# NikolaZubic/2dimageto3dmodel

Measured on NVIDIA H100. Metric: render+loss+GAN images/sec (cfg3: cfg2 render+loss at batch 32 + conv-GAN 256x256 G/D iteration, 1 G : 2 D, Adam), higher is better.
Workload: dtype tf32 (convs) / f32

## Files before the change

2dimageto3dmodel_b200/csrc/b3d_core.cu:

```cuda
#include <atomic>
#include <stdarg.h>
#include <string.h>

#include "b3d_common.cuh"

namespace b3d {
static thread_local char g_err[512] = "";
static thread_local char g_variant[256] = "";
static std::atomic<uint64_t> g_launches{0};

void set_error(const char* fmt, ...) {
    va_list ap;
    va_start(ap, fmt);
    vsnprintf(g_err, sizeof(g_err), fmt, ap);
    va_end(ap);
}
void clear_variant() { g_variant[0] = 0; }
void add_variant(const char* fmt, ...) {
    size_t n = strlen(g_variant);
    if (n + 2 >= sizeof(g_variant)) return;
    if (n) g_variant[n++] = ';';
    va_list ap;
    va_start(ap, fmt);
    vsnprintf(g_variant + n, sizeof(g_variant) - n, fmt, ap);
    va_end(ap);
}
void count_launch(int n) { g_launches.fetch_add((uint64_t)n, std::memory_order_relaxed); }
}

extern "C" {
const char* b3d_last_error(void) { return b3d::g_err; }
const char* b3d_last_variant(void) { return b3d::g_variant; }
int b3d_version(void) { return 410; }
uint64_t b3d_launch_count(void) { return b3d::g_launches.load(std::memory_order_relaxed); }
}
```

2dimageto3dmodel_b200/csrc/tc_common.cuh:

```cuda
#pragma once
#include <cuda.h>
#include <cuda_runtime.h>
#include <stdint.h>

#include "b3d_common.cuh"

namespace tc {

__device__ __forceinline__ uint32_t smem_u32(const void* p) { return (uint32_t)__cvta_generic_to_shared(p); }

__device__ __forceinline__ void mbar_init(uint64_t* bar, uint32_t count) {
    asm volatile("mbarrier.init.shared::cta.b64 [%0], %1;" ::"r"(smem_u32(bar)), "r"(count));
}
__device__ __forceinline__ void fence_barrier_init() { asm volatile("fence.mbarrier_init.release.cluster;" ::: "memory"); }
__device__ __forceinline__ void fence_proxy_async() { asm volatile("fence.proxy.async.shared::cta;" ::: "memory"); }

__device__ __forceinline__ void mbar_arrive_expect_tx(uint64_t* bar, uint32_t bytes) {
    asm volatile("mbarrier.arrive.expect_tx.shared::cta.b64 _, [%0], %1;" ::"r"(smem_u32(bar)), "r"(bytes) : "memory");
}
__device__ __forceinline__ void mbar_arrive(uint64_t* bar) {
    asm volatile("mbarrier.arrive.shared::cta.b64 _, [%0];" ::"r"(smem_u32(bar)) : "memory");
}
__device__ __forceinline__ void mbar_arrive(uint64_t* bar, uint32_t count) {
    asm volatile("mbarrier.arrive.shared::cta.b64 _, [%0], %1;" ::"r"(smem_u32(bar)), "r"(count) : "memory");
}
__device__ __forceinline__ void mbar_wait(uint64_t* bar, uint32_t parity) {
    asm volatile(
        "{\n"
        ".reg .pred p;\n"
        "WAIT_LOOP:\n"
        "mbarrier.try_wait.parity.shared::cta.b64 p, [%0], %1;\n"
        "@p bra WAIT_DONE;\n"
        "bra WAIT_LOOP;\n"
        "WAIT_DONE:\n"
        "}\n" ::"r"(smem_u32(bar)),
        "r"(parity)
        : "memory");
}
__device__ __forceinline__ void named_sync(uint32_t id, uint32_t count) {
    asm volatile("bar.sync %0, %1;" ::"r"(id), "r"(count) : "memory");
}

__device__ __forceinline__ void tma_prefetch_desc(const CUtensorMap* m) {
    asm volatile("prefetch.tensormap [%0];" ::"l"(reinterpret_cast<uint64_t>(m)) : "memory");
}
__device__ __forceinline__ void tma_load_3d(void* smem, const CUtensorMap* m, uint64_t* bar, int c0, int c1, int c2) {
    asm volatile(
        "cp.async.bulk.tensor.3d.shared::cluster.global.mbarrier::complete_tx::bytes [%0], [%1, {%3, %4, %5}], [%2];" ::"r"(
            smem_u32(smem)),
        "l"(reinterpret_cast<uint64_t>(m)), "r"(smem_u32(bar)), "r"(c0), "r"(c1), "r"(c2)
        : "memory");
}
__device__ __forceinline__ void tma_load_4d(void* smem, const CUtensorMap* m, uint64_t* bar, int c0, int c1, int c2,
                                            int c3) {
    asm volatile(
        "cp.async.bulk.tensor.4d.shared::cluster.global.mbarrier::complete_tx::bytes [%0], [%1, {%3, %4, %5, %6}], "
        "[%2];" ::"r"(smem_u32(smem)),
        "l"(reinterpret_cast<uint64_t>(m)), "r"(smem_u32(bar)), "r"(c0), "r"(c1), "r"(c2), "r"(c3)
        : "memory");
}
__device__ __forceinline__ void tma_load_5d(void* smem, const CUtensorMap* m, uint64_t* bar, int c0, int c1, int c2,
                                            int c3, int c4) {
    asm volatile(
        "cp.async.bulk.tensor.5d.shared::cluster.global.mbarrier::complete_tx::bytes [%0], [%1, {%3, %4, %5, %6, %7}], "
        "[%2];" ::"r"(smem_u32(smem)),
        "l"(reinterpret_cast<uint64_t>(m)), "r"(smem_u32(bar)), "r"(c0), "r"(c1), "r"(c2), "r"(c3), "r"(c4)
        : "memory");
}

__device__ __forceinline__ void wgmma_fence() { asm volatile("wgmma.fence.sync.aligned;" ::: "memory"); }
__device__ __forceinline__ void wgmma_commit() { asm volatile("wgmma.commit_group.sync.aligned;" ::: "memory"); }
template <int N>
__device__ __forceinline__ void wgmma_wait() { asm volatile("wgmma.wait_group.sync.aligned %0;" ::"n"(N) : "memory"); }
__device__ __forceinline__ uint32_t lds_u32(uint32_t smem_addr) {
    uint32_t v;
    asm volatile("ld.shared.b32 %0, [%1];" : "=r"(v) : "r"(smem_addr) : "memory");
    return v;
}
__device__ __forceinline__ float lds_f32(uint32_t smem_addr) {
    float v;
    asm volatile("ld.shared.f32 %0, [%1];" : "=f"(v) : "r"(smem_addr) : "memory");
    return v;
}
__device__ __forceinline__ float2 lds_f32x2(uint32_t smem_addr) {
    float2 v;
    asm volatile("ld.shared.v2.f32 {%0, %1}, [%2];" : "=f"(v.x), "=f"(v.y) : "r"(smem_addr) : "memory");
    return v;
}
template <int N>
__device__ __forceinline__ void setmaxnreg_dec() { asm volatile("setmaxnreg.dec.sync.aligned.u32 %0;" ::"n"(N)); }
template <int N>
__device__ __forceinline__ void setmaxnreg_inc() { asm volatile("setmaxnreg.inc.sync.aligned.u32 %0;" ::"n"(N)); }

template <int N>
struct Wgmma;
template <>
struct Wgmma<64> {
    __device__ __forceinline__ static void mma_rs(float (&d)[32], const uint32_t (&a)[4], uint64_t db, uint32_t accumulate) {
        asm volatile(
            "{\n"
            ".reg .pred p;\n"
            "setp.ne.b32 p, %37, 0;\n"
            "wgmma.mma_async.sync.aligned.m64n64k8.f32.tf32.tf32 "
            "{%0, %1, %2, %3, %4, %5, %6, %7, %8, %9, %10, %11, %12, %13, %14, %15, %16, %17, %18, %19, %20, %21, %22, %23, %24, %25, %26, %27, %28, %29, %30, %31}, "
            "{%32, %33, %34, %35}, %36, p, 1, 1;\n"
            "}\n"
            : "+f"(d[0]), "+f"(d[1]), "+f"(d[2]), "+f"(d[3]), "+f"(d[4]), "+f"(d[5]), "+f"(d[6]), "+f"(d[7]), "+f"(d[8]), "+f"(d[9]), "+f"(d[10]), "+f"(d[11]), "+f"(d[12]), "+f"(d[13]), "+f"(d[14]), "+f"(d[15]), "+f"(d[16]), "+f"(d[17]), "+f"(d[18]), "+f"(d[19]), "+f"(d[20]), "+f"(d[21]), "+f"(d[22]), "+f"(d[23]), "+f"(d[24]), "+f"(d[25]), "+f"(d[26]), "+f"(d[27]), "+f"(d[28]), "+f"(d[29]), "+f"(d[30]), "+f"(d[31])
            : "r"(a[0]), "r"(a[1]), "r"(a[2]), "r"(a[3]), "l"(db), "r"(accumulate));
    }
    __device__ __forceinline__ static void mma(float (&d)[32], uint64_t da, uint64_t db, uint32_t accumulate) {
        asm volatile(
            "{\n"
            ".reg .pred p;\n"
            "setp.ne.b32 p, %34, 0;\n"
            "wgmma.mma_async.sync.aligned.m64n64k8.f32.tf32.tf32 "
            "{%0, %1, %2, %3, %4, %5, %6, %7, %8, %9, %10, %11, %12, %13, %14, %15, %16, %17, %18, %19, %20, %21, %22, %23, %24, %25, %26, %27, %28, %29, %30, %31}, "
            "%32, %33, p, 1, 1;\n"
            "}\n"
            : "+f"(d[0]), "+f"(d[1]), "+f"(d[2]), "+f"(d[3]), "+f"(d[4]), "+f"(d[5]), "+f"(d[6]), "+f"(d[7]), "+f"(d[8]), "+f"(d[9]), "+f"(d[10]), "+f"(d[11]), "+f"(d[12]), "+f"(d[13]), "+f"(d[14]), "+f"(d[15]), "+f"(d[16]), "+f"(d[17]), "+f"(d[18]), "+f"(d[19]), "+f"(d[20]), "+f"(d[21]), "+f"(d[22]), "+f"(d[23]), "+f"(d[24]), "+f"(d[25]), "+f"(d[26]), "+f"(d[27]), "+f"(d[28]), "+f"(d[29]), "+f"(d[30]), "+f"(d[31])
            : "l"(da), "l"(db), "r"(accumulate));
    }
};
template <>
struct Wgmma<128> {
    __device__ __forceinline__ static void mma_rs(float (&d)[64], const uint32_t (&a)[4], uint64_t db, uint32_t accumulate) {
        asm volatile(
            "{\n"
            ".reg .pred p;\n"
            "setp.ne.b32 p, %69, 0;\n"
            "wgmma.mma_async.sync.aligned.m64n128k8.f32.tf32.tf32 "
            "{%0, %1, %2, %3, %4, %5, %6, %7, %8, %9, %10, %11, %12, %13, %14, %15, %16, %17, %18, %19, %20, %21, %22, %23, %24, %25, %26, %27, %28, %29, %30, %31, %32, %33, %34, %35, %36, %37, %38, %39, %40, %41, %42, %43, %44, %45, %46, %47, %48, %49, %50, %51, %52, %53, %54, %55, %56, %57, %58, %59, %60, %61, %62, %63}, "
            "{%64, %65, %66, %67}, %68, p, 1, 1;\n"
            "}\n"
            : "+f"(d[0]), "+f"(d[1]), "+f"(d[2]), "+f"(d[3]), "+f"(d[4]), "+f"(d[5]), "+f"(d[6]), "+f"(d[7]), "+f"(d[8]), "+f"(d[9]), "+f"(d[10]), "+f"(d[11]), "+f"(d[12]), "+f"(d[13]), "+f"(d[14]), "+f"(d[15]), "+f"(d[16]), "+f"(d[17]), "+f"(d[18]), "+f"(d[19]), "+f"(d[20]), "+f"(d[21]), "+f"(d[22]), "+f"(d[23]), "+f"(d[24]), "+f"(d[25]), "+f"(d[26]), "+f"(d[27]), "+f"(d[28]), "+f"(d[29]), "+f"(d[30]), "+f"(d[31]), "+f"(d[32]), "+f"(d[33]), "+f"(d[34]), "+f"(d[35]), "+f"(d[36]), "+f"(d[37]), "+f"(d[38]), "+f"(d[39]), "+f"(d[40]), "+f"(d[41]), "+f"(d[42]), "+f"(d[43]), "+f"(d[44]), "+f"(d[45]), "+f"(d[46]), "+f"(d[47]), "+f"(d[48]), "+f"(d[49]), "+f"(d[50]), "+f"(d[51]), "+f"(d[52]), "+f"(d[53]), "+f"(d[54]), "+f"(d[55]), "+f"(d[56]), "+f"(d[57]), "+f"(d[58]), "+f"(d[59]), "+f"(d[60]), "+f"(d[61]), "+f"(d[62]), "+f"(d[63])
            : "r"(a[0]), "r"(a[1]), "r"(a[2]), "r"(a[3]), "l"(db), "r"(accumulate));
    }
    __device__ __forceinline__ static void mma(float (&d)[64], uint64_t da, uint64_t db, uint32_t accumulate) {
        asm volatile(
            "{\n"
            ".reg .pred p;\n"
            "setp.ne.b32 p, %66, 0;\n"
            "wgmma.mma_async.sync.aligned.m64n128k8.f32.tf32.tf32 "
            "{%0, %1, %2, %3, %4, %5, %6, %7, %8, %9, %10, %11, %12, %13, %14, %15, %16, %17, %18, %19, %20, %21, %22, %23, %24, %25, %26, %27, %28, %29, %30, %31, %32, %33, %34, %35, %36, %37, %38, %39, %40, %41, %42, %43, %44, %45, %46, %47, %48, %49, %50, %51, %52, %53, %54, %55, %56, %57, %58, %59, %60, %61, %62, %63}, "
            "%64, %65, p, 1, 1;\n"
            "}\n"
            : "+f"(d[0]), "+f"(d[1]), "+f"(d[2]), "+f"(d[3]), "+f"(d[4]), "+f"(d[5]), "+f"(d[6]), "+f"(d[7]), "+f"(d[8]), "+f"(d[9]), "+f"(d[10]), "+f"(d[11]), "+f"(d[12]), "+f"(d[13]), "+f"(d[14]), "+f"(d[15]), "+f"(d[16]), "+f"(d[17]), "+f"(d[18]), "+f"(d[19]), "+f"(d[20]), "+f"(d[21]), "+f"(d[22]), "+f"(d[23]), "+f"(d[24]), "+f"(d[25]), "+f"(d[26]), "+f"(d[27]), "+f"(d[28]), "+f"(d[29]), "+f"(d[30]), "+f"(d[31]), "+f"(d[32]), "+f"(d[33]), "+f"(d[34]), "+f"(d[35]), "+f"(d[36]), "+f"(d[37]), "+f"(d[38]), "+f"(d[39]), "+f"(d[40]), "+f"(d[41]), "+f"(d[42]), "+f"(d[43]), "+f"(d[44]), "+f"(d[45]), "+f"(d[46]), "+f"(d[47]), "+f"(d[48]), "+f"(d[49]), "+f"(d[50]), "+f"(d[51]), "+f"(d[52]), "+f"(d[53]), "+f"(d[54]), "+f"(d[55]), "+f"(d[56]), "+f"(d[57]), "+f"(d[58]), "+f"(d[59]), "+f"(d[60]), "+f"(d[61]), "+f"(d[62]), "+f"(d[63])
            : "l"(da), "l"(db), "r"(accumulate));
    }
};
__device__ __forceinline__ uint64_t desc_k128(uint32_t smem_addr) {
    uint64_t d = 0;
    d |= (uint64_t)((smem_addr & 0x3FFFF) >> 4);
    d |= (uint64_t)1 << 16;
    d |= (uint64_t)(1024 >> 4) << 32;
    d |= (uint64_t)1 << 62;
    return d;
}
__device__ __forceinline__ uint64_t desc_k32(uint32_t smem_addr) {
    uint64_t d = 0;
    d |= (uint64_t)((smem_addr & 0x3FFFF) >> 4);
    d |= (uint64_t)1 << 16;
    d |= (uint64_t)(256 >> 4) << 32;
    d |= (uint64_t)3 << 62;
    return d;
}

__device__ __forceinline__ void transpose_slice_k128(const float* raw, unsigned char* dst, int rows, int tid, int blk_stride = 1024,
                                                     int k0 = 0) {
    for (int i = tid; i < rows * 8; i += 128) {
        const int mn = i % rows, kc = i / rows;
        const float* src = raw + (mn >> 5) * blk_stride + (k0 + kc * 4) * 32 + (mn & 31);
        const float4 v = make_float4(src[0], src[32], src[64], src[96]);
        *reinterpret_cast<float4*>(dst + mn * 128 + ((kc ^ (mn & 7)) << 4)) = v;
    }
}

typedef CUresult (*EncodeTiledFn)(CUtensorMap*, CUtensorMapDataType, cuuint32_t, void*, const cuuint64_t*,
                                  const cuuint64_t*, const cuuint32_t*, const cuuint32_t*, CUtensorMapInterleave,
                                  CUtensorMapSwizzle, CUtensorMapL2promotion, CUtensorMapFloatOOBfill);

inline EncodeTiledFn encode_fn() {
    static EncodeTiledFn fn = nullptr;
    if (!fn) {
        void* p = nullptr;
        cudaDriverEntryPointQueryResult q;
        if (cudaGetDriverEntryPoint("cuTensorMapEncodeTiled", &p, cudaEnableDefault, &q) == cudaSuccess &&
            q == cudaDriverEntryPointSuccess)
            fn = reinterpret_cast<EncodeTiledFn>(p);
    }
    return fn;
}

inline int make_tmap_f32(CUtensorMap* m, const void* base, int rank, const uint64_t* dims, const uint64_t* strides_b,
                         const uint32_t* box, const uint32_t* elem_strides = nullptr,
                         CUtensorMapSwizzle swz = CU_TENSOR_MAP_SWIZZLE_128B) {
    EncodeTiledFn fn = encode_fn();
    if (!fn) {
        b3d::set_error("cuTensorMapEncodeTiled is not available from the driver");
        return B3D_ECUDA;
    }
    cuuint64_t gd[5], gs[5];
    cuuint32_t bx[5], es[5];
    for (int i = 0; i < rank; ++i) {
        gd[i] = dims[i];
        bx[i] = box[i];
        es[i] = elem_strides ? elem_strides[i] : 1;
        if (i > 0) gs[i - 1] = strides_b[i - 1];
    }
    CUresult r = fn(m, CU_TENSOR_MAP_DATA_TYPE_FLOAT32, (cuuint32_t)rank, const_cast<void*>(base), gd, gs, bx, es,
                    CU_TENSOR_MAP_INTERLEAVE_NONE, swz, CU_TENSOR_MAP_L2_PROMOTION_L2_256B,
                    CU_TENSOR_MAP_FLOAT_OOB_FILL_NONE);
    if (r != CUDA_SUCCESS) {
        b3d::set_error("cuTensorMapEncodeTiled failed with CUresult %d (rank %d, inner box %u)", (int)r, rank, box[0]);
        return B3D_ECUDA;
    }
    return B3D_OK;
}

inline int num_sms() {
    int dev = 0, n = 0;
    if (cudaGetDevice(&dev) != cudaSuccess || cudaDeviceGetAttribute(&n, cudaDevAttrMultiProcessorCount, dev) != cudaSuccess || n < 1)
        return 132;
    return n;
}

}
```

2dimageto3dmodel_b200/csrc/tc_conv.cu:

```cuda
#include "tc_common.cuh"

namespace {

constexpr int BM = 128;
constexpr int BK = 32;
constexpr int MMA_K = 8;
constexpr int MAX_TAPS = 25;
constexpr int NTHREADS = 384;

struct ConvParams {
    int N, Hout, Wout, Cout;
    int BW, BH, BI;
    int tiles_x, tiles_y;
    int xbase;
    int ntaps, kslices;
    int sy, sx;
    int dy[MAX_TAPS], dx[MAX_TAPS];
    int wtap[MAX_TAPS];
    int OH, OW, OC, osy, osx;
    float leaky;
    double* stats;
    int fold;
    int fold_y0;
    int mask;
// ... 146 lines not shown
            sq[e] += __shfl_xor_sync(0xffffffffu, sq[e], 2);
            if ((lane & 3) == 0 && cok[e]) {
                atomicAdd(p.stats + c0 + cw + 8 * e, (double)sum[e]);
                if (!p.stats_sum) atomicAdd(p.stats + p.Cout + c0 + cw + 8 * e, (double)sq[e]);
            }
        }
    }
}

constexpr int PRODUCER_REGS = 24, CONSUMER_REGS = 240;

template <int BN, int STAGES, int KW>
__global__ void __launch_bounds__(NTHREADS, 1)
conv_wgmma_kernel(const __grid_constant__ CUtensorMap tmap_x, const __grid_constant__ CUtensorMap tmap_w,
                  const __grid_constant__ CUtensorMap tmap_m, const ConvParams p, const float* __restrict__ bias,
                  float* __restrict__ out, int tiles, int work_items) {
    using S = CSmem<BN, STAGES, KW>;
    constexpr bool COOP = kCoop<BN>;
    constexpr int OWNERS = COOP ? 1 : 2;
    constexpr int G = kMaskGroup<BN>;
    static_assert(G <= STAGES, "the mask stages of one block do not fit the ring");
    extern __shared__ unsigned char smem_raw[];
    unsigned char* base = reinterpret_cast<unsigned char*>((reinterpret_cast<uintptr_t>(smem_raw) + 1023) & ~uintptr_t(1023));
    uint64_t* full = reinterpret_cast<uint64_t*>(base + STAGES * S::STAGE_BYTES);
    uint64_t* empty = full + OWNERS * STAGES;
    static_assert((OWNERS + 1) * STAGES * 8 <= 256, "barriers do not fit their area");
    if (threadIdx.x == 0) {
        tc::tma_prefetch_desc(&tmap_x);
        tc::tma_prefetch_desc(&tmap_w);
        if (p.mask) tc::tma_prefetch_desc(&tmap_m);
        for (int s = 0; s < STAGES; ++s) {
            for (int o = 0; o < OWNERS; ++o) tc::mbar_init(full + o * STAGES + s, 1);
            tc::mbar_init(empty + s, kEmptyArrivals<BN>);
        }
        tc::fence_barrier_init();
    }
    __syncthreads();
    const int KI = p.ntaps / KW * p.kslices;
    const int MS = p.mask ? BN / 32 : 0;
    const int wg = threadIdx.x >> 7;

    if (wg == 0) {
        tc::setmaxnreg_dec<PRODUCER_REGS>();
        if (threadIdx.x == 0) {
            uint32_t git = 0;
            for (int w = blockIdx.x, k = 0; w < work_items; w += gridDim.x, ++k) {
                uint64_t* fb = full + (COOP ? 0 : (k & 1) * STAGES);
                const int cls = w % p.ncls, wq = w / p.ncls, tb = cls * p.ntaps;
                int t = wq % tiles;
                const int c0 = (wq / tiles) * BN;
                const int x0 = p.xbase + (t % p.tiles_x) * p.BW;
                t /= p.tiles_x;
                const int y0 = (t % p.tiles_y) * p.BH, n0 = (t / p.tiles_y) * p.BI;
                for (int it = 0; it < KI; ++it, ++git) {
                    const int s = git % STAGES;
                    tc::mbar_wait(empty + s, ((git / STAGES) & 1) ^ 1);
                    const int tap = it / p.kslices * KW, ks = it % p.kslices;
                    unsigned char* a = base + s * S::STAGE_BYTES;
                    tc::mbar_arrive_expect_tx(fb + s, S::TX_BYTES);
                    if (KW > 1)
                        tc::tma_load_4d(a, &tmap_x, fb + s, ks * BK, x0 + p.dx0, y0 + p.dy[tb + tap], n0);
                    else if (p.fold)
                        tc::tma_load_4d(a, &tmap_x, fb + s, 0, x0 + p.dx[tb + tap], y0 + p.fold_y0 + 4 * ks, n0);
                    else
                        tc::tma_load_4d(a, &tmap_x, fb + s, ks * BK, p.sx * x0 + p.dx[tb + tap], p.sy * y0 + p.dy[tb + tap], n0);
                    tc::tma_load_3d(a + S::A_BYTES, &tmap_w, fb + s, ks * BK, c0, p.wtap[tb + tap]);
                }
                const int mx = p.osx * x0 + p.coox[cls], my = p.osy * y0 + p.cooy[cls];
                for (int m = 0; m < MS; ++m, ++git) {
                    const int s = git % STAGES;
                    tc::mbar_wait(empty + s, ((git / STAGES) & 1) ^ 1);
                    tc::mbar_arrive_expect_tx(fb + s, MASK_BYTES);
                    tc::tma_load_4d(base + s * S::STAGE_BYTES, &tmap_m, fb + s, c0 + mask_chunk_channel(m, G), mx, my, n0);
                }
            }
        }
        return;
    }
    tc::setmaxnreg_inc<CONSUMER_REGS>();

    const int h = wg - 1, tid = threadIdx.x & 127, lane = tid & 31;
    float acc[kBlocks<BN>][BM / 2];
#pragma unroll
    for (int m = 0; m < kBlocks<BN>; ++m)
#pragma unroll
        for (int i = 0; i < BM / 2; ++i) acc[m][i] = 0.f;
    uint32_t git = 0, phase = 0;
    const uint32_t ring = tc::smem_u32(base);
    TileAt at;
    at.lbw = __ffs(p.BW) - 1;
    at.lbwh = at.lbw + __ffs(p.BH) - 1;
    uint64_t* fb = full + (COOP ? 0 : h * STAGES);
    const int cb = COOP ? 128 * h : 0;
    const int cw = (tid >> 5) * 16 + (lane >> 2);
    const int mine = (COOP ? 2 * h : 0) + (tid >> 6);
    for (int k = COOP ? 0 : h;; k += COOP ? 1 : 2) {
        const int w = blockIdx.x + k * gridDim.x;
        if (w >= work_items) break;
        git = (uint32_t)k * (KI + MS);
        const int wq = w / p.ncls, tile = wq % tiles, c0 = (wq / tiles) * BN + cb;
        tile_origin(p, at, tile, w % p.ncls);
        if (KW == 1 && p.fold) mainloop<BN, STAGES, KW, true>(acc, base, fb, empty, KI, git, phase, cb, tid == 0, p.shift);
        else mainloop<BN, STAGES, KW, false>(acc, base, fb, empty, KI, git, phase, cb, tid == 0, p.shift);
        uint32_t neg[kBlocks<BN>][2] = {};
        if (p.mask) {
#pragma unroll
            for (int m = 0; m < kBlocks<BN>; ++m, git += G) {
                uint32_t mstage = 0;
#pragma unroll
                for (int i = 0; i < G; ++i) {
                    const int s = (git + i) % STAGES;
                    tc::mbar_wait(fb + s, (phase >> s) & 1);
                    phase ^= 1u << s;
                    if (i == mine) mstage = ring + s * S::STAGE_BYTES;
                }
                mask_bits<G, STAGES>(neg[m], mstage, cw, lane, empty, git);
            }
        }
#pragma unroll
        for (int m = 0; m < kBlocks<BN>; ++m) {
            if (p.mask) epilogue_block<true>(acc[m], neg[m], p, at, bias, out, c0 + 64 * m, cw, lane);
            else epilogue_block<false>(acc[m], neg[m], p, at, bias, out, c0 + 64 * m, cw, lane);
        }
    }
}

struct WgradParams {
    int N, Hout, Wout, Cout, Cin;
    int BWk, BHk;
    int kx, ky;
    int kh, kw, pad_y, st;
    int xoff;
    int splits;
    int tapmajor;
    int tstep;
};

template <int BN, int STAGES, int NRAW, int T>
struct WSmem {
    static constexpr int DY_BYTES = BM * BK * 4;
    static constexpr int STAGE_BYTES = T * BN * BK * 4;
    static constexpr int WROWS = T == 1 ? 32 : 36;
    static constexpr int RAW_X = (BN / 32) * WROWS * 128;
    static constexpr int RAW_BYTES = (DY_BYTES + RAW_X + 1023) / 1024 * 1024;
    static constexpr int TOTAL = STAGES * STAGE_BYTES + NRAW * RAW_BYTES + 1024 + 256;
};

__host__ __device__ constexpr int wgrad_row_co(int m) { return (m & 35) | ((m & 8) >> 1) | ((m & 16) >> 1) | ((m & 4) << 2); }

__host__ __device__ constexpr int dy_tile_offset(int co, int px) {
    return (co >> 5) * 4096 + px * 128 + ((((co >> 2) & 7) ^ (px & 7)) << 4) + (co & 3) * 4;
}

template <int BN, int STAGES, int NRAW, int T>
__global__ void __launch_bounds__(NTHREADS, 1)
wgrad_wgmma_kernel(const __grid_constant__ CUtensorMap tmap_dy, const __grid_constant__ CUtensorMap tmap_x,
                   const WgradParams p, float* __restrict__ dw) {
    using S = WSmem<BN, STAGES, NRAW, T>;
    extern __shared__ unsigned char smem_raw[];
    unsigned char* base = reinterpret_cast<unsigned char*>((reinterpret_cast<uintptr_t>(smem_raw) + 1023) & ~uintptr_t(1023));
    unsigned char* raw = base + STAGES * S::STAGE_BYTES;
    uint64_t* full = reinterpret_cast<uint64_t*>(raw + NRAW * S::RAW_BYTES);
    uint64_t* empty = full + STAGES;
    uint64_t* rawfull = empty + STAGES;
    uint64_t* rawempty = rawfull + NRAW;

    const int co0 = blockIdx.x * BM, ci0 = blockIdx.y * BN;
    const int gpr = p.kw / T;
    const int groups = p.kh * gpr;
    const int grp = blockIdx.z % groups, split = blockIdx.z / groups;
    const int r = grp / gpr, s = grp % gpr;
    const int per_img = p.kx * p.ky;
    const long long ktotal = (long long)p.N * per_img;
    const long long k_lo = ktotal * split / p.splits, k_hi = ktotal * (split + 1) / p.splits;
    const int KI = (int)(k_hi - k_lo);

    if (threadIdx.x == 0) {
        tc::tma_prefetch_desc(&tmap_dy);
        tc::tma_prefetch_desc(&tmap_x);
        for (int i = 0; i < STAGES; ++i) {
            tc::mbar_init(full + i, 128);
            tc::mbar_init(empty + i, 2);
        }
        for (int i = 0; i < NRAW; ++i) {
            tc::mbar_init(rawfull + i, 1);
            tc::mbar_init(rawempty + i, 8);
        }
        tc::fence_barrier_init();
    }
    __syncthreads();
    const int wg = threadIdx.x >> 7, tid = threadIdx.x & 127;

    if (wg == 0) {
        tc::setmaxnreg_dec<56>();
        auto issue = [&](int j) {
            if (tid != 0) return;
            const long long k = k_lo + j;
            const int n = (int)(k / per_img), rem = (int)(k % per_img);
            const int x0 = (rem % p.kx) * p.BWk, y0 = (rem / p.kx) * p.BHk;
            const int rb = j % NRAW;
            unsigned char* dst = raw + rb * S::RAW_BYTES;
            tc::mbar_wait(rawempty + rb, ((j / NRAW) & 1) ^ 1);
            tc::mbar_arrive_expect_tx(rawfull + rb, S::DY_BYTES + S::RAW_X);
            tc::tma_load_5d(dst, &tmap_dy, rawfull + rb, 0, x0, y0, n, co0 / 32);
            tc::tma_load_5d(dst + S::DY_BYTES, &tmap_x, rawfull + rb, 0, p.st * x0 + s + p.xoff, p.st * y0 + r - p.pad_y, n, ci0 / 32);
        };
        for (int j = 0; j < NRAW - 1 && j < KI; ++j) issue(j);
        for (int it = 0; it < KI; ++it) {
            if (it + NRAW - 1 < KI) issue(it + NRAW - 1);
            const int rb = it % NRAW, st = it % STAGES;
            tc::mbar_wait(rawfull + rb, (it / NRAW) & 1);
            tc::mbar_wait(empty + st, ((it / STAGES) & 1) ^ 1);
            const float* src = reinterpret_cast<const float*>(raw + rb * S::RAW_BYTES + S::DY_BYTES);
            unsigned char* dst = base + st * S::STAGE_BYTES;
#pragma unroll
            for (int t = 0; t < T; ++t)
                tc::transpose_slice_k128(src, dst + t * (BN * 128), BN, tid, S::WROWS * 32, t);
            tc::fence_proxy_async();
            tc::mbar_arrive(full + st);
            tc::named_sync(2, 128);
        }
        return;
    }
    tc::setmaxnreg_inc<224>();

    const int h = wg - 1, lane = tid & 31;
    int aoff[4];
#pragma unroll
    for (int e = 0; e < 4; ++e)
        aoff[e] = dy_tile_offset(h * 64 + wgrad_row_co((tid >> 5) * 16 + (lane >> 2) + 8 * (e & 1)), (lane & 3) + 4 * (e >> 1));
    float acc[T][BN / 2];
#pragma unroll
    for (int t = 0; t < T; ++t)
#pragma unroll
        for (int i = 0; i < BN / 2; ++i) acc[t][i] = 0.f;
    const uint32_t raw_s = tc::smem_u32(raw);
    for (int it = 0; it < KI; ++it) {
        const int st = it % STAGES, rb = it % NRAW;
        tc::mbar_wait(rawfull + rb, (it / NRAW) & 1);
        uint32_t frag[BK / MMA_K][4];
#pragma unroll
        for (int k = 0; k < BK / MMA_K; ++k)
#pragma unroll
            for (int e = 0; e < 4; ++e) frag[k][e] = tc::lds_u32(raw_s + rb * S::RAW_BYTES + aoff[e] + k * 1024);
        __syncwarp();
        if (lane == 0) tc::mbar_arrive(rawempty + rb);
        tc::mbar_wait(full + st, (it / STAGES) & 1);
        const uint32_t b = tc::smem_u32(base + st * S::STAGE_BYTES);
        tc::wgmma_fence();
#pragma unroll
        for (int t = 0; t < T; ++t)
#pragma unroll
            for (int k = 0; k < BK / MMA_K; ++k)
                tc::Wgmma<BN>::mma_rs(acc[t], frag[k], tc::desc_k128(b + t * (BN * 128) + k * MMA_K * 4), (it | k) ? 1u : 0u);
        tc::wgmma_commit();
        tc::wgmma_wait<0>();
        if (tid == 0) tc::mbar_arrive(empty + st);
    }
    if (KI == 0) return;
    const int m_a = (tid >> 5) * 16 + (lane >> 2);
    const int cq = ci0 + 2 * (lane & 3);
#pragma unroll
    for (int t = 0; t < T; ++t) {
        const int sc = s + t * p.tstep;
#pragma unroll
        for (int e = 0; e < 2; ++e) {
            const int co = co0 + h * 64 + wgrad_row_co(m_a + 8 * e);
            if (co >= p.Cout) continue;
#pragma unroll
            for (int j = 0; j < BN / 8; ++j) {
                const int ci = cq + 8 * j;
                if (ci >= p.Cin) continue;
                const float v0 = acc[t][4 * j + 2 * e], v1 = acc[t][4 * j + 2 * e + 1];
                if (p.tapmajor) {
                    atomicAdd(reinterpret_cast<float2*>(dw + ((size_t)(r * p.kw + sc) * p.Cout + co) * p.Cin + ci), make_float2(v0, v1));
                } else {
                    atomicAdd(dw + (((size_t)co * p.Cin + ci) * p.kh + r) * p.kw + sc, v0);
                    atomicAdd(dw + (((size_t)co * p.Cin + ci + 1) * p.kh + r) * p.kw + sc, v1);
                }
            }
        }
    }
}

template <int BN, int STAGES, int NRAW, int T>
int launch_wgrad(const CUtensorMap& mdy, const CUtensorMap& mx, const WgradParams& p, float* dw, dim3 grid, cudaStream_t st) {
    using S = WSmem<BN, STAGES, NRAW, T>;
    static_assert(S::TOTAL <= 227 * 1024, "wgrad pipeline does not fit shared memory");
    B3D_CUDA_OK(cudaFuncSetAttribute(wgrad_wgmma_kernel<BN, STAGES, NRAW, T>, cudaFuncAttributeMaxDynamicSharedMemorySize, S::TOTAL));
    wgrad_wgmma_kernel<BN, STAGES, NRAW, T><<<grid, NTHREADS, S::TOTAL, st>>>(mdy, mx, p, dw);
    B3D_LAUNCH_OK();
    b3d::add_variant("wgrad_wgmma<%d,%d,%d,%d>", BN, STAGES, NRAW, T);
    return B3D_OK;
}

constexpr int STEM_KW = 5, STEM_STAGES = 4, STEM_NRAW = 3;
struct StemSmem {
    static constexpr int DY_BYTES = 64 * BK * 4;
    static constexpr int WPX = BK + STEM_KW - 1;
    static constexpr int RAW_X_MAX = 8 * WPX * 32;
    static constexpr int RAW_BYTES = (DY_BYTES + RAW_X_MAX + 1023) / 1024 * 1024;
    static constexpr int TILE_BYTES = 64 * BK * 4;
    static constexpr int STAGE_BYTES = STEM_KW * TILE_BYTES;
    static constexpr int TOTAL = STEM_STAGES * STAGE_BYTES + STEM_NRAW * RAW_BYTES + 1024 + 256;
};

__global__ void __launch_bounds__(NTHREADS, 1)
wgrad_stem_kernel(const __grid_constant__ CUtensorMap tmap_dy, const __grid_constant__ CUtensorMap tmap_x,
                  const WgradParams p, int fold_kh, float* __restrict__ dw) {
    using S = StemSmem;
    extern __shared__ unsigned char smem_raw[];
    unsigned char* base = reinterpret_cast<unsigned char*>((reinterpret_cast<uintptr_t>(smem_raw) + 1023) & ~uintptr_t(1023));
    unsigned char* raw = base + STEM_STAGES * S::STAGE_BYTES;
    uint64_t* full = reinterpret_cast<uint64_t*>(raw + STEM_NRAW * S::RAW_BYTES);
    uint64_t* empty = full + STEM_STAGES;
    uint64_t* rawfull = empty + STEM_STAGES;
    uint64_t* rawempty = rawfull + STEM_NRAW;

    const int co0 = blockIdx.x * 64, split = blockIdx.y;
    const int per_img = p.kx * p.ky;
    const long long ktotal = (long long)p.N * per_img;
    const long long k_lo = ktotal * split / p.splits, k_hi = ktotal * (split + 1) / p.splits;
    const int KI = (int)(k_hi - k_lo);
    const int creal = 8 * fold_kh;
    const int xbytes = fold_kh * S::WPX * 32;

    if (threadIdx.x == 0) {
        tc::tma_prefetch_desc(&tmap_dy);
        tc::tma_prefetch_desc(&tmap_x);
        for (int i = 0; i < STEM_STAGES; ++i) {
            tc::mbar_init(full + i, 128);
            tc::mbar_init(empty + i, 1);
        }
        for (int i = 0; i < STEM_NRAW; ++i) {
            tc::mbar_init(rawfull + i, 1);
            tc::mbar_init(rawempty + i, 4);
        }
        tc::fence_barrier_init();
    }
    __syncthreads();
    const int wg = threadIdx.x >> 7, tid = threadIdx.x & 127;

    if (wg == 0) {
        tc::setmaxnreg_dec<56>();
        auto issue = [&](int j) {
            if (tid != 0) return;
            const long long k = k_lo + j;
            const int n = (int)(k / per_img), rem = (int)(k % per_img);
            const int x0 = (rem % p.kx) * BK, y0 = rem / p.kx;
            const int rb = j % STEM_NRAW;
            unsigned char* dst = raw + rb * S::RAW_BYTES;
            tc::mbar_wait(rawempty + rb, ((j / STEM_NRAW) & 1) ^ 1);
            tc::mbar_arrive_expect_tx(rawfull + rb, S::DY_BYTES + xbytes);
            tc::tma_load_5d(dst, &tmap_dy, rawfull + rb, 0, x0, y0, n, co0 / 32);
            tc::tma_load_4d(dst + S::DY_BYTES, &tmap_x, rawfull + rb, 0, x0, y0 - p.pad_y, n);
        };
        for (int i = tid; i < STEM_STAGES * STEM_KW * (64 - creal) * 8; i += 128) {
            const int c = creal + (i >> 3) % (64 - creal), tile = (i >> 3) / (64 - creal);
            *reinterpret_cast<float4*>(base + tile * S::TILE_BYTES + c * 128 + (i & 7) * 16) = make_float4(0.f, 0.f, 0.f, 0.f);
        }
        for (int j = 0; j < STEM_NRAW - 1 && j < KI; ++j) issue(j);
        const int ntask = fold_kh * 8 * STEM_KW * 8;
        for (int it = 0; it < KI; ++it) {
            if (it + STEM_NRAW - 1 < KI) issue(it + STEM_NRAW - 1);
            const int rb = it % STEM_NRAW, st = it % STEM_STAGES;
            tc::mbar_wait(rawfull + rb, (it / STEM_NRAW) & 1);
            tc::mbar_wait(empty + st, ((it / STEM_STAGES) & 1) ^ 1);
            const float* src = reinterpret_cast<const float*>(raw + rb * S::RAW_BYTES + S::DY_BYTES);
            unsigned char* dst = base + st * S::STAGE_BYTES;
            for (int i = tid; i < ntask; i += 128) {
                const int ci = i & 7, u = i >> 3;
                const int s = u % STEM_KW, q = (u / STEM_KW) & 7, r = u / (STEM_KW * 8);
                const float* a = src + (r * S::WPX + 4 * q + s) * 8 + ci;
                const int c = 8 * r + ci;
                *reinterpret_cast<float4*>(dst + s * S::TILE_BYTES + c * 128 + ((q ^ ci) << 4)) = make_float4(a[0], a[8], a[16], a[24]);
            }
            tc::fence_proxy_async();
            tc::mbar_arrive(full + st);
            tc::named_sync(2, 128);
        }
        return;
    }
    tc::setmaxnreg_inc<224>();

    const int h = wg - 1, lane = tid & 31;
    int aoff[4];
#pragma unroll
    for (int e = 0; e < 4; ++e)
        aoff[e] = dy_tile_offset(wgrad_row_co((tid >> 5) * 16 + (lane >> 2) + 8 * (e & 1)), (lane & 3) + 4 * (e >> 1));
    float acc[STEM_KW][32];
#pragma unroll
    for (int t = 0; t < STEM_KW; ++t)
#pragma unroll
        for (int i = 0; i < 32; ++i) acc[t][i] = 0.f;
    const uint32_t raw_s = tc::smem_u32(raw);
    for (int it = h; it < KI; it += 2) {
        const int st = it % STEM_STAGES, rb = it % STEM_NRAW;
        tc::mbar_wait(rawfull + rb, (it / STEM_NRAW) & 1);
        uint32_t frag[BK / MMA_K][4];
#pragma unroll
        for (int k = 0; k < BK / MMA_K; ++k)
#pragma unroll
            for (int e = 0; e < 4; ++e) frag[k][e] = tc::lds_u32(raw_s + rb * S::RAW_BYTES + aoff[e] + k * 1024);
        __syncwarp();
        if (lane == 0) tc::mbar_arrive(rawempty + rb);
        tc::mbar_wait(full + st, (it / STEM_STAGES) & 1);
        const uint32_t b = tc::smem_u32(base + st * S::STAGE_BYTES);
        tc::wgmma_fence();
#pragma unroll
        for (int t = 0; t < STEM_KW; ++t)
#pragma unroll
            for (int k = 0; k < BK / MMA_K; ++k)
                tc::Wgmma<64>::mma_rs(acc[t], frag[k], tc::desc_k128(b + t * S::TILE_BYTES + k * MMA_K * 4), 1u);
        tc::wgmma_commit();
        tc::wgmma_wait<0>();
        if (tid == 0) tc::mbar_arrive(empty + st);
    }
    if (h >= KI) return;
    const int m_a = (tid >> 5) * 16 + (lane >> 2);
#pragma unroll
    for (int t = 0; t < STEM_KW; ++t) {
#pragma unroll
        for (int e = 0; e < 2; ++e) {
            const int co = co0 + wgrad_row_co(m_a + 8 * e);
#pragma unroll
            for (int j = 0; j < 8; ++j) {
                const int ci = 8 * j + 2 * (lane & 3);
                if (ci >= creal) continue;
                const float v0 = acc[t][4 * j + 2 * e], v1 = acc[t][4 * j + 2 * e + 1];
                if (p.tapmajor) {
                    atomicAdd(reinterpret_cast<float2*>(dw + ((size_t)t * p.Cout + co) * p.Cin + ci), make_float2(v0, v1));
                } else {
                    atomicAdd(dw + ((size_t)co * p.Cin + ci) * STEM_KW + t, v0);
                    atomicAdd(dw + ((size_t)co * p.Cin + ci + 1) * STEM_KW + t, v1);
                }
            }
        }
    }
}

int wgrad_splits(int base_ctas, long long ktotal) {
    constexpr long long FIXED = 16;
    const long long sms = tc::num_sms();
    long long smax = ktotal / 8;
    if (smax > 8 * sms) smax = 8 * sms;
    int best = 1;
    long long best_cost = -1;
    for (long long s = 1; s <= smax; ++s) {
        const long long cost = (base_ctas * s + sms - 1) / sms * ((ktotal + s - 1) / s + FIXED);
        if (best_cost < 0 || cost < best_cost) { best = (int)s; best_cost = cost; }
    }
    return best;
}

template <int BN, int STAGES, int KW = 1>
int launch_conv(const CUtensorMap& mx, const CUtensorMap& mw, const CUtensorMap& mm, const ConvParams& p, const float* bias, float* out,
                int tiles, cudaStream_t st) {
    using S = CSmem<BN, STAGES, KW>;
    static_assert(S::TOTAL <= 227 * 1024, "conv pipeline does not fit shared memory");
    B3D_CUDA_OK(cudaFuncSetAttribute(conv_wgmma_kernel<BN, STAGES, KW>, cudaFuncAttributeMaxDynamicSharedMemorySize, S::TOTAL));
    const int work = tiles * b3d::ceil_div(p.Cout, BN) * p.ncls;
    const int sms = tc::num_sms();
    conv_wgmma_kernel<BN, STAGES, KW><<<work < sms ? work : sms, NTHREADS, S::TOTAL, st>>>(mx, mw, mm, p, bias, out, tiles, work);
    B3D_LAUNCH_OK();
    if (KW > 1) b3d::add_variant("conv_wgmma_rowwin<%d,%d,%d>", BN, KW, STAGES);
    else b3d::add_variant("conv_wgmma<%d,%d>", BN, STAGES);
    return B3D_OK;
}

template <int BN>
int launch_rowwin(int kw, const CUtensorMap& mx, const CUtensorMap& mw, const CUtensorMap& mm, const ConvParams& p, const float* bias,
                  float* out, int tiles, cudaStream_t st) {
    if (kw == 2) return launch_conv<BN, BN == 64 ? 5 : 4, 2>(mx, mw, mm, p, bias, out, tiles, st);
    if (kw == 3) return launch_conv<BN, BN == 64 ? 4 : 3, 3>(mx, mw, mm, p, bias, out, tiles, st);
    return launch_conv<BN, BN == 64 ? 3 : 2, 5>(mx, mw, mm, p, bias, out, tiles, st);
}

int pow2_floor(int v) {
    int p = 1;
    while (p * 2 <= v) p *= 2;
    return p;
}

}

extern "C" {

int b3d_conv2d_tf32(const float* x, const float* wt, const float* bias, float* out, int N, int H, int W, int Cin,
                    int Hout, int Wout, int Cout, int ntaps, const int* dy, const int* dx, int sy, int sx, int OH,
                    int OW, int OC, int osy, int osx, int ooy, int oox, float leaky, const int* wtap,
                    int wtaps_total, double* stats, int fold_kh, int fold_pad, const b3d_conv_opts* opts, void* stream) {
    B3D_REQUIRE(N > 0 && H > 0 && W > 0 && Hout > 0 && Wout > 0 && Cout > 0, B3D_EINVAL, "b3d_conv2d_tf32: bad sizes");
    B3D_REQUIRE(Cin > 0 && Cin % BK == 0, B3D_EINVAL, "b3d_conv2d_tf32: Cin=%d must be a multiple of %d", Cin, BK);
    B3D_REQUIRE(ntaps >= 1 && ntaps <= MAX_TAPS && dy && dx, B3D_EINVAL, "b3d_conv2d_tf32: bad taps");
    B3D_REQUIRE(x && wt && out, B3D_EINVAL, "b3d_conv2d_tf32: null pointer");
    B3D_REQUIRE(sy >= 1 && sy <= 2 && sx >= 1 && sx <= 2, B3D_EINVAL, "b3d_conv2d_tf32: stride must be 1 or 2");
    if (!wtap) wtaps_total = ntaps;
    B3D_REQUIRE(wtaps_total >= ntaps || wtap, B3D_EINVAL, "b3d_conv2d_tf32: bad weight tap count");
    for (int t = 0; wtap && t < ntaps; ++t)
        B3D_REQUIRE(wtap[t] >= 0 && wtap[t] < wtaps_total, B3D_EINVAL, "b3d_conv2d_tf32: weight tap %d out of range", wtap[t]);
    B3D_CHECK_ALIGNED(x);
    B3D_CHECK_ALIGNED(wt);
    b3d::clear_variant();

    const float* mask = opts ? opts->mask : nullptr;
    const float mslope = opts ? opts->mask_slope : 1.f;
    B3D_REQUIRE(!mask || (reinterpret_cast<uintptr_t>(mask) % 16 == 0 && OC % 4 == 0), B3D_EINVAL,
                "b3d_conv2d_tf32: the mask needs a 16-byte aligned base and OC %% 4 == 0 (OC=%d)", OC);
    const int stats_sum = (opts && opts->stats_sum_only) ? 1 : 0;
    const int xpitch = (opts && opts->x_row_pitch) ? opts->x_row_pitch : W;
    const int ncls = (opts && opts->nclass > 1) ? opts->nclass : 1;
    B3D_REQUIRE(ncls <= 4 && ntaps % ncls == 0 && (ncls == 1 || (sy == 1 && sx == 1 && fold_kh == 0)), B3D_EINVAL,
                "b3d_conv2d_tf32: nclass=%d needs <= 4 equal tap groups of a stride-1 launch", ncls);
    const int tpc = ntaps / ncls;
    int cooy[4] = {ooy, ooy, ooy, ooy}, coox[4] = {oox, oox, oox, oox};
    for (int c = 0; c < ncls && ncls > 1; ++c) { cooy[c] = opts->class_ooy[c]; coox[c] = opts->class_oox[c]; }
    B3D_REQUIRE(xpitch >= W && (fold_kh == 0 || xpitch == W), B3D_EINVAL, "b3d_conv2d_tf32: x_row_pitch=%d must be >= W=%d (and absent with the on-the-fly fold)", xpitch, W);
    if (fold_kh > 0) {
        B3D_REQUIRE(fold_kh <= 8 && Cin == 32 * ((8 * fold_kh + 31) / 32) && sy == 1 && sx == 1 && !wtap && Wout % BM == 0,
                    B3D_EINVAL, "b3d_conv2d_tf32: on-the-fly fold needs 8 input channels, stride 1 and Wout %% 128 == 0 (Wout=%d)", Wout);
    }
    B3D_REQUIRE(!stats || mask || (osy == 1 && osx == 1), B3D_EINVAL, "b3d_conv2d_tf32: statistics need a dense output");
    const bool bn256 = Cout % 256 == 0 && (long long)N * Hout * Wout / BM * (Cout / 256) * ncls >= tc::num_sms();
    const int BN = bn256 ? 256 : Cout > 64 ? 128 : 64;
    cudaStream_t st = (cudaStream_t)stream;
    CUtensorMap mw;
    {
        const uint64_t dims[3] = {(uint64_t)Cin, (uint64_t)Cout, (uint64_t)wtaps_total};
        const uint64_t strides[2] = {(uint64_t)Cin * 4, (uint64_t)Cout * Cin * 4};
        const uint32_t box[3] = {(uint32_t)BK, (uint32_t)BN, 1};
        if (int rc = tc::make_tmap_f32(&mw, wt, 3, dims, strides, box)) return rc;
    }

    int g_kw = 0, g_step = 1, g_wstep = 1;
    if (sy == 1 && sx == 1 && fold_kh == 0) {
        int kw_ = 1;
        while (kw_ < tpc && dy[kw_] == dy[0]) ++kw_;
        const int step = kw_ > 1 ? dx[1] - dx[0] : 1;
        const int wstep = (wtap && kw_ > 1) ? wtap[1] - wtap[0] : 1;
        bool grid_ok = tpc % kw_ == 0 && (kw_ == 2 || kw_ == 3 || kw_ == 5) && (step == 1 || step == -1) && wstep >= 1 && wstep <= 2 &&
                       (ncls == 1 || wtap != nullptr);
        for (int t = 0; grid_ok && t < ntaps; ++t) {
            const int tc_ = t % tpc, t0 = t - tc_;
            grid_ok = dy[t] == dy[t0 + (tc_ / kw_) * kw_] && dx[t] == dx[0] + (tc_ % kw_) * step;
            if (wtap) grid_ok = grid_ok && wtap[t] == wtap[t0 + (tc_ / kw_) * kw_] + (tc_ % kw_) * wstep;
        }
        if (grid_ok && BN <= 128) { g_kw = kw_; g_step = step; g_wstep = wstep; }
    }

    auto run = [&](int xlo, int xhi) -> int {
        const int wspan = xhi - xlo;
        ConvParams p{};
        p.N = N; p.Hout = Hout; p.Wout = xhi; p.Cout = Cout; p.xbase = xlo;
        p.BW = pow2_floor(wspan < BM ? wspan : BM);
        p.BH = pow2_floor(Hout < BM / p.BW ? Hout : BM / p.BW);
        p.BI = BM / (p.BW * p.BH);
        p.tiles_x = b3d::ceil_div(wspan, p.BW);
        p.tiles_y = b3d::ceil_div(Hout, p.BH);
        const int tiles = p.tiles_x * p.tiles_y * b3d::ceil_div(N, p.BI);
        p.ntaps = tpc; p.kslices = Cin / BK; p.sy = sy; p.sx = sx; p.ncls = ncls;
        for (int t = 0; t < ntaps; ++t) { p.dy[t] = dy[t]; p.dx[t] = dx[t]; p.wtap[t] = wtap ? wtap[t] : t; }
        for (int c = 0; c < 4; ++c) { p.cooy[c] = cooy[c]; p.coox[c] = coox[c]; }
        p.OH = OH; p.OW = OW; p.OC = OC; p.osy = osy; p.osx = osx;
        p.leaky = leaky;
        p.stats = stats;
        p.mask = mask != nullptr; p.mslope = mslope; p.stats_sum = stats_sum;
        p.fold = fold_kh; p.fold_y0 = -fold_pad;
        {
            const unsigned long long esn = p.BI > 1 ? (unsigned long long)OH * OW * OC : 0, esy = p.BH > 1 ? (unsigned long long)osy * OW * OC : 0,
                                     esx = (unsigned long long)osx * OC;
// ... 143 lines not shown
```

Baseline: 1382.

## Pipeline wgrad wgmma consumers and vectorize producer transposes in weight-gradient kernels

Consumer warpgroups in the wgrad and stem kernels now go through a shared helper that double-buffers A fragments and keeps one wgmma group in flight (wait<1>), releasing each stage one iteration later. The producer transposes are rewritten as batched vectorized shared-memory loads and stores with a new swizzle mapping. An idle second consumer warpgroup now exits early when Cout fits in one 64-row half, and the register split is rebalanced between producer and consumers. The aim is to overlap MMA with fragment loads and speed up the producer transpose, at the cost of more register pressure and more complex barrier accounting.

```diff
diff --git a/2dimageto3dmodel_b200/csrc/b3d_core.cu b/2dimageto3dmodel_b200/csrc/b3d_core.cu
--- a/2dimageto3dmodel_b200/csrc/b3d_core.cu
+++ b/2dimageto3dmodel_b200/csrc/b3d_core.cu
@@ -31,6 +31,6 @@
 extern "C" {
 const char* b3d_last_error(void) { return b3d::g_err; }
 const char* b3d_last_variant(void) { return b3d::g_variant; }
-int b3d_version(void) { return 410; }
+int b3d_version(void) { return 420; }
 uint64_t b3d_launch_count(void) { return b3d::g_launches.load(std::memory_order_relaxed); }
 }
diff --git a/2dimageto3dmodel_b200/csrc/tc_common.cuh b/2dimageto3dmodel_b200/csrc/tc_common.cuh
--- a/2dimageto3dmodel_b200/csrc/tc_common.cuh
+++ b/2dimageto3dmodel_b200/csrc/tc_common.cuh
@@ -87,6 +87,16 @@
     asm volatile("ld.shared.v2.f32 {%0, %1}, [%2];" : "=f"(v.x), "=f"(v.y) : "r"(smem_addr) : "memory");
     return v;
 }
+__device__ __forceinline__ float4 lds_f32x4(uint32_t smem_addr) {
+    float4 v;
+    asm volatile("ld.shared.v4.f32 {%0, %1, %2, %3}, [%4];" : "=f"(v.x), "=f"(v.y), "=f"(v.z), "=f"(v.w) : "r"(smem_addr) : "memory");
+    return v;
+}
+__device__ __forceinline__ void sts_f32x4(uint32_t smem_addr, float a, float b, float c, float d) {
+    asm volatile("st.shared.v4.f32 [%0], {%1, %2, %3, %4};" ::"r"(smem_addr), "f"(a), "f"(b), "f"(c), "f"(d) : "memory");
+}
+__device__ __forceinline__ void fence_operand(uint32_t& r) { asm volatile("" : "+r"(r)::"memory"); }
+__device__ __forceinline__ void fence_operand(float& r) { asm volatile("" : "+f"(r)::"memory"); }
 template <int N>
 __device__ __forceinline__ void setmaxnreg_dec() { asm volatile("setmaxnreg.dec.sync.aligned.u32 %0;" ::"n"(N)); }
 template <int N>
@@ -165,16 +175,6 @@
     return d;
 }
 
-__device__ __forceinline__ void transpose_slice_k128(const float* raw, unsigned char* dst, int rows, int tid, int blk_stride = 1024,
-                                                     int k0 = 0) {
-    for (int i = tid; i < rows * 8; i += 128) {
-        const int mn = i % rows, kc = i / rows;
-        const float* src = raw + (mn >> 5) * blk_stride + (k0 + kc * 4) * 32 + (mn & 31);
-        const float4 v = make_float4(src[0], src[32], src[64], src[96]);
-        *reinterpret_cast<float4*>(dst + mn * 128 + ((kc ^ (mn & 7)) << 4)) = v;
-    }
-}
-
 typedef CUresult (*EncodeTiledFn)(CUtensorMap*, CUtensorMapDataType, cuuint32_t, void*, const cuuint64_t*,
                                   const cuuint64_t*, const cuuint32_t*, const cuuint32_t*, CUtensorMapInterleave,
                                   CUtensorMapSwizzle, CUtensorMapL2promotion, CUtensorMapFloatOOBfill);
diff --git a/2dimageto3dmodel_b200/csrc/tc_conv.cu b/2dimageto3dmodel_b200/csrc/tc_conv.cu
--- a/2dimageto3dmodel_b200/csrc/tc_conv.cu
+++ b/2dimageto3dmodel_b200/csrc/tc_conv.cu
@@ -322,6 +322,89 @@
     return (co >> 5) * 4096 + px * 128 + ((((co >> 2) & 7) ^ (px & 7)) << 4) + (co & 3) * 4;
 }
 
+__host__ __device__ constexpr int xt_chunk(int i) { return (((i & 7) >> 1) ^ ((i >> 4) & 3)) | (((i >> 3) & 1) << 2); }
+__host__ __device__ constexpr int xt_src_offset(int i, int px, int wrows) { return ((i >> 6) * wrows + px) * 128 + (i & 7) * 16; }
+__host__ __device__ constexpr int xt_dst_offset(int i, int j) {
+    return ((i >> 6) * 32 + 4 * (i & 7) + j) * 128 + ((xt_chunk(i) ^ ((4 * (i & 7) + j) & 7)) << 4);
+}
+template <int BN, int T, int WROWS>
+__device__ __forceinline__ void wgrad_transpose(uint32_t src, uint32_t dst, int tid) {
+    constexpr int NT = 2 * BN / 128;
+    float4 v[NT][T + 3];
+#pragma unroll
+    for (int n = 0; n < NT; ++n)
+#pragma unroll
+        for (int u = 0; u < T + 3; ++u) v[n][u] = tc::lds_f32x4(src + xt_src_offset(tid + 128 * n, 4 * xt_chunk(tid + 128 * n) + u, WROWS));
+#pragma unroll
+    for (int n = 0; n < NT; ++n) {
+        const int i = tid + 128 * n;
+#pragma unroll
+        for (int t = 0; t < T; ++t) {
+            const uint32_t d = dst + t * (BN * 128);
+            const float4* w = v[n] + t;
+            tc::sts_f32x4(d + xt_dst_offset(i, 0), w[0].x, w[1].x, w[2].x, w[3].x);
+            tc::sts_f32x4(d + xt_dst_offset(i, 1), w[0].y, w[1].y, w[2].y, w[3].y);
+            tc::sts_f32x4(d + xt_dst_offset(i, 2), w[0].z, w[1].z, w[2].z, w[3].z);
+            tc::sts_f32x4(d + xt_dst_offset(i, 3), w[0].w, w[1].w, w[2].w, w[3].w);
+        }
+    }
+}
+
+template <int N, int T, int STAGES, int NRAW, int RAW_BYTES, int STAGE_BYTES>
+__device__ __forceinline__ void wgrad_consume(float (&acc)[T][N / 2], uint32_t raw_s, uint32_t stage_s, uint64_t* full,
+                                              uint64_t* empty, uint64_t* rawfull, uint64_t* rawempty, const int (&aoff)[4],
+                                              int first, int step, int KI, int tid, bool zero_first) {
+    using Frag = uint32_t[BK / MMA_K][4];
+    auto load = [&](Frag& f, int j) {
+        const int rb = j % NRAW;
+        tc::mbar_wait(rawfull + rb, (j / NRAW) & 1);
+#pragma unroll
+        for (int k = 0; k < BK / MMA_K; ++k)
+#pragma unroll
+            for (int e = 0; e < 4; ++e) f[k][e] = tc::lds_u32(raw_s + rb * RAW_BYTES + aoff[e] + k * 1024);
+        __syncwarp();
+        if ((tid & 31) == 0) tc::mbar_arrive(rawempty + rb);
+    };
+    auto slice = [&](int j, Frag& f, Frag& g) {
+        const int st = j % STAGES;
+        tc::mbar_wait(full + st, (j / STAGES) & 1);
+        const uint32_t b = stage_s + st * STAGE_BYTES;
+        tc::wgmma_fence();
+#pragma unroll
+        for (int t = 0; t < T; ++t)
+#pragma unroll
+            for (int k = 0; k < BK / MMA_K; ++k)
+                tc::Wgmma<N>::mma_rs(acc[t], f[k], tc::desc_k128(b + t * (N * 128) + k * MMA_K * 4), (zero_first && j == first && k == 0) ? 0u : 1u);
+        tc::wgmma_commit();
+        tc::wgmma_wait<1>();
+#pragma unroll
+        for (int k = 0; k < BK / MMA_K; ++k)
+#pragma unroll
+            for (int e = 0; e < 4; ++e) tc::fence_operand(g[k][e]);
+        if (j != first && tid == 0) tc::mbar_arrive(empty + (j - step) % STAGES);
+        if (j + step < KI) load(g, j + step);
+    };
+    Frag f0, f1;
+    if (first < KI) load(f0, first);
+    for (int j = first; j < KI; j += 2 * step) {
+        slice(j, f0, f1);
+        if (j + step < KI) slice(j + step, f1, f0);
+    }
+    tc::wgmma_wait<0>();
+#pragma unroll
+    for (int k = 0; k < BK / MMA_K; ++k)
+#pragma unroll
+        for (int e = 0; e < 4; ++e) {
+            tc::fence_operand(f0[k][e]);
+            tc::fence_operand(f1[k][e]);
+        }
+#pragma unroll
+    for (int t = 0; t < T; ++t)
+#pragma unroll
+        for (int i = 0; i < N / 2; ++i) tc::fence_operand(acc[t][i]);
+    if (first < KI && tid == 0) tc::mbar_arrive(empty + (first + (KI - 1 - first) / step * step) % STAGES);
+}
+
 template <int BN, int STAGES, int NRAW, int T>
 __global__ void __launch_bounds__(NTHREADS, 1)
 wgrad_wgmma_kernel(const __grid_constant__ CUtensorMap tmap_dy, const __grid_constant__ CUtensorMap tmap_x,
@@ -344,17 +427,18 @@
     const long long ktotal = (long long)p.N * per_img;
     const long long k_lo = ktotal * split / p.splits, k_hi = ktotal * (split + 1) / p.splits;
     const int KI = (int)(k_hi - k_lo);
+    const int nact = co0 + 64 < p.Cout ? 2 : 1;
 
     if (threadIdx.x == 0) {
         tc::tma_prefetch_desc(&tmap_dy);
         tc::tma_prefetch_desc(&tmap_x);
         for (int i = 0; i < STAGES; ++i) {
             tc::mbar_init(full + i, 128);
-            tc::mbar_init(empty + i, 2);
+            tc::mbar_init(empty + i, nact);
         }
         for (int i = 0; i < NRAW; ++i) {
             tc::mbar_init(rawfull + i, 1);
-            tc::mbar_init(rawempty + i, 8);
+            tc::mbar_init(rawempty + i, 4 * nact);
         }
         tc::fence_barrier_init();
     }
@@ -362,7 +446,7 @@
     const int wg = threadIdx.x >> 7, tid = threadIdx.x & 127;
 
     if (wg == 0) {
-        tc::setmaxnreg_dec<56>();
+        tc::setmaxnreg_dec<80>();
         auto issue = [&](int j) {
             if (tid != 0) return;
             const long long k = k_lo + j;
@@ -376,25 +460,23 @@
             tc::tma_load_5d(dst + S::DY_BYTES, &tmap_x, rawfull + rb, 0, p.st * x0 + s + p.xoff, p.st * y0 + r - p.pad_y, n, ci0 / 32);
         };
         for (int j = 0; j < NRAW - 1 && j < KI; ++j) issue(j);
+        const uint32_t raw_s = tc::smem_u32(raw), base_s = tc::smem_u32(base);
         for (int it = 0; it < KI; ++it) {
             if (it + NRAW - 1 < KI) issue(it + NRAW - 1);
             const int rb = it % NRAW, st = it % STAGES;
             tc::mbar_wait(rawfull + rb, (it / NRAW) & 1);
             tc::mbar_wait(empty + st, ((it / STAGES) & 1) ^ 1);
-            const float* src = reinterpret_cast<const float*>(raw + rb * S::RAW_BYTES + S::DY_BYTES);
-            unsigned char* dst = base + st * S::STAGE_BYTES;
-#pragma unroll
-            for (int t = 0; t < T; ++t)
-                tc::transpose_slice_k128(src, dst + t * (BN * 128), BN, tid, S::WROWS * 32, t);
+            wgrad_transpose<BN, T, S::WROWS>(raw_s + rb * S::RAW_BYTES + S::DY_BYTES, base_s + st * S::STAGE_BYTES, tid);
             tc::fence_proxy_async();
             tc::mbar_arrive(full + st);
             tc::named_sync(2, 128);
         }
         return;
     }
-    tc::setmaxnreg_inc<224>();
+    tc::setmaxnreg_inc<208>();
 
     const int h = wg - 1, lane = tid & 31;
+    if (h >= nact) return;
     int aoff[4];
 #pragma unroll
     for (int e = 0; e < 4; ++e)
@@ -404,29 +486,8 @@
     for (int t = 0; t < T; ++t)
 #pragma unroll
         for (int i = 0; i < BN / 2; ++i) acc[t][i] = 0.f;
-    const uint32_t raw_s = tc::smem_u32(raw);
-    for (int it = 0; it < KI; ++it) {
-        const int st = it % STAGES, rb = it % NRAW;
-        tc::mbar_wait(rawfull + rb, (it / NRAW) & 1);
-        uint32_t frag[BK / MMA_K][4];
-#pragma unroll
-        for (int k = 0; k < BK / MMA_K; ++k)
-#pragma unroll
-            for (int e = 0; e < 4; ++e) frag[k][e] = tc::lds_u32(raw_s + rb * S::RAW_BYTES + aoff[e] + k * 1024);
-        __syncwarp();
-        if (lane == 0) tc::mbar_arrive(rawempty + rb);
-        tc::mbar_wait(full + st, (it / STAGES) & 1);
-        const uint32_t b = tc::smem_u32(base + st * S::STAGE_BYTES);
-        tc::wgmma_fence();
-#pragma unroll
-        for (int t = 0; t < T; ++t)
-#pragma unroll
-            for (int k = 0; k < BK / MMA_K; ++k)
-                tc::Wgmma<BN>::mma_rs(acc[t], frag[k], tc::desc_k128(b + t * (BN * 128) + k * MMA_K * 4), (it | k) ? 1u : 0u);
-        tc::wgmma_commit();
-        tc::wgmma_wait<0>();
-        if (tid == 0) tc::mbar_arrive(empty + st);
-    }
+    wgrad_consume<BN, T, STAGES, NRAW, S::RAW_BYTES, S::STAGE_BYTES>(acc, tc::smem_u32(raw), tc::smem_u32(base), full, empty, rawfull,
+                                                                     rawempty, aoff, 0, 1, KI, tid, true);
     if (KI == 0) return;
     const int m_a = (tid >> 5) * 16 + (lane >> 2);
     const int cq = ci0 + 2 * (lane & 3);
@@ -465,6 +526,7 @@
 }
 
 constexpr int STEM_KW = 5, STEM_STAGES = 4, STEM_NRAW = 3;
+constexpr int STEM_BATCH = 3;
 struct StemSmem {
     static constexpr int DY_BYTES = 64 * BK * 4;
     static constexpr int WPX = BK + STEM_KW - 1;
@@ -531,19 +593,33 @@
         }
         for (int j = 0; j < STEM_NRAW - 1 && j < KI; ++j) issue(j);
         const int ntask = fold_kh * 8 * STEM_KW * 8;
+        const uint32_t raw_s = tc::smem_u32(raw), base_s = tc::smem_u32(base);
         for (int it = 0; it < KI; ++it) {
             if (it + STEM_NRAW - 1 < KI) issue(it + STEM_NRAW - 1);
             const int rb = it % STEM_NRAW, st = it % STEM_STAGES;
             tc::mbar_wait(rawfull + rb, (it / STEM_NRAW) & 1);
             tc::mbar_wait(empty + st, ((it / STEM_STAGES) & 1) ^ 1);
-            const float* src = reinterpret_cast<const float*>(raw + rb * S::RAW_BYTES + S::DY_BYTES);
-            unsigned char* dst = base + st * S::STAGE_BYTES;
-            for (int i = tid; i < ntask; i += 128) {
-                const int ci = i & 7, u = i >> 3;
-                const int s = u % STEM_KW, q = (u / STEM_KW) & 7, r = u / (STEM_KW * 8);
-                const float* a = src + (r * S::WPX + 4 * q + s) * 8 + ci;
-                const int c = 8 * r + ci;
-                *reinterpret_cast<float4*>(dst + s * S::TILE_BYTES + c * 128 + ((q ^ ci) << 4)) = make_float4(a[0], a[8], a[16], a[24]);
+            const uint32_t src = raw_s + rb * S::RAW_BYTES + S::DY_BYTES;
+            const uint32_t dst = base_s + st * S::STAGE_BYTES;
+            for (int i0 = tid; i0 < ntask; i0 += STEM_BATCH * 128) {
+                float v[STEM_BATCH][4];
+                uint32_t d[STEM_BATCH];
+#pragma unroll
+                for (int g = 0; g < STEM_BATCH; ++g) {
+                    const int i = i0 + 128 * g;
+                    if (i >= ntask) break;
+                    const int ci = i & 7, u = i >> 3;
+                    const int s = u % STEM_KW, q = (u / STEM_KW) & 7, r = u / (STEM_KW * 8);
+                    const uint32_t a = src + ((r * S::WPX + 4 * q + s) * 8 + ci) * 4;
+#pragma unroll
+                    for (int e = 0; e < 4; ++e) v[g][e] = tc::lds_f32(a + 32 * e);
+                    d[g] = dst + s * S::TILE_BYTES + (8 * r + ci) * 128 + ((q ^ ci) << 4);
+                }
+#pragma unroll
+                for (int g = 0; g < STEM_BATCH; ++g) {
+                    if (i0 + 128 * g >= ntask) break;
+                    tc::sts_f32x4(d[g], v[g][0], v[g][1], v[g][2], v[g][3]);
+                }
             }
             tc::fence_proxy_async();
             tc::mbar_arrive(full + st);
@@ -563,29 +639,9 @@
     for (int t = 0; t < STEM_KW; ++t)
 #pragma unroll
         for (int i = 0; i < 32; ++i) acc[t][i] = 0.f;
-    const uint32_t raw_s = tc::smem_u32(raw);
-    for (int it = h; it < KI; it += 2) {
-        const int st = it % STEM_STAGES, rb = it % STEM_NRAW;
-        tc::mbar_wait(rawfull + rb, (it / STEM_NRAW) & 1);
-        uint32_t frag[BK / MMA_K][4];
-#pragma unroll
-        for (int k = 0; k < BK / MMA_K; ++k)
-#pragma unroll
-            for (int e = 0; e < 4; ++e) frag[k][e] = tc::lds_u32(raw_s + rb * S::RAW_BYTES + aoff[e] + k * 1024);
-        __syncwarp();
-        if (lane == 0) tc::mbar_arrive(rawempty + rb);
-        tc::mbar_wait(full + st, (it / STEM_STAGES) & 1);
-        const uint32_t b = tc::smem_u32(base + st * S::STAGE_BYTES);
-        tc::wgmma_fence();
-#pragma unroll
-        for (int t = 0; t < STEM_KW; ++t)
-#pragma unroll
-            for (int k = 0; k < BK / MMA_K; ++k)
-                tc::Wgmma<64>::mma_rs(acc[t], frag[k], tc::desc_k128(b + t * S::TILE_BYTES + k * MMA_K * 4), 1u);
-        tc::wgmma_commit();
-        tc::wgmma_wait<0>();
-        if (tid == 0) tc::mbar_arrive(empty + st);
-    }
+    static_assert(S::TILE_BYTES == 64 * 128, "a tap's B tile is 64 channel rows of 128 bytes");
+    wgrad_consume<64, STEM_KW, STEM_STAGES, STEM_NRAW, S::RAW_BYTES, S::STAGE_BYTES>(acc, tc::smem_u32(raw), tc::smem_u32(base), full, empty,
+                                                                                     rawfull, rawempty, aoff, h, 2, KI, tid, false);
     if (h >= KI) return;
     const int m_a = (tid >> 5) * 16 + (lane >> 2);
 #pragma unroll
```

After: 1442 (median of 6 runs). 4.3% higher.
